# ambicuity/Distributed-LLM-Training-and-Inference-System

Hardware: AMD Instinct MI355X
Metric: tokens/sec (node) GPT-7B train (higher is better)
Workload: dtype bf16; 1 GPU; model=gpt-7b, global_batch=16, seq_len=2048, parallelism=dp1, micro_batch=16, grad_accum=1, activation_checkpoint=none, layout=planner

## Files before the change

### llmctl/config/knobs.py

```python

from __future__ import annotations

import contextlib
import dataclasses
import os
from dataclasses import dataclass, fields
from typing import Any, Dict, Iterator, Optional

ENV = "LLMCTL_KNOBS"


@dataclass(frozen=True)
class PerfKnobs:
    gemm64: bool = True
    gemm64_config: int = 304
    fwd64: str = "auto"
    dgrad64: str = "fused"
    wgrad_kernel: bool = True
    swiglu_bwd: str = "side"
    dgrad_transpose: bool = True
    wt_side_stream: bool = True
    fused_fwd: bool = False
    rope_inplace: bool = True
    fused_rope_attn: bool = True
    moe_pad: bool = True
    overlap_optimizer: bool = False
    gemm_tuning: bool = True
    fa_split: int = -1
    fa_prio: int = 1
    fa_nw: int = 4
    dkv: int = 2
    dkv_nwg: int = 0
    async_tp: bool = True
    async_tp_save_full: bool = False
    cp_zigzag: bool = True
    decode_fused: bool = True
    decode_splits: int = 0
    decode_v3: int = 1
    skinny_gemm: str = "auto"
    prefill_swiglu: bool = True
    prefill_fa: bool = True
    prefill_norm_fold: bool = True
    mixed_steps: bool = True
    custom_ar: bool = True
    tp_graphs: bool = True
    async_decode: bool = True
    tp_fused_decode: bool = True

    def as_dict(self) -> Dict[str, Any]:
        return dataclasses.asdict(self)


NATIVE = ("fa_split", "fa_prio", "fa_nw", "dkv", "dkv_nwg", "decode_splits", "decode_v3")
_FIELDS = {f.name: f for f in fields(PerfKnobs)}


def _coerce(name: str, value: Any) -> Any:
    if name not in _FIELDS:
        raise KeyError(f"unknown performance knob {name!r} (known: {', '.join(sorted(_FIELDS))})")
    typ = _FIELDS[name].type
    if typ in ("bool", bool):
        if isinstance(value, str):
            v = value.strip().lower()
            if v not in ("1", "0", "true", "false", "on", "off", "yes", "no"):
                raise ValueError(f"knob {name}: expected a boolean, got {value!r}")
            return v in ("1", "true", "on", "yes")
        return bool(value)
    if typ in ("int", int):
        return int(value)
    return str(value)


def parse_env(spec: Optional[str]) -> Dict[str, Any]:
    out: Dict[str, Any] = {}
    for part in (spec or "").split(","):
        part = part.strip()
        if not part:
            continue
        if "=" not in part:
            raise ValueError(f"{ENV}: expected name=value, got {part!r}")
        k, v = part.split("=", 1)
        out[k.strip()] = _coerce(k.strip(), v.strip())
    return out


_RETIRED_ENV = ("LLMCTL_SIDE_DGRAD", "LLMCTL_DECODE_ATTN_QKV", "LLMCTL_GEMM64_CONFIG", "LLMCTL_SKINNY")
_warned: set = set()


def _warn_retired_env() -> None:
    import warnings

    names = [f"LLMCTL_{n.upper()}" for n in _FIELDS] + list(_RETIRED_ENV)
    for n in names:
        if n in os.environ and n not in _warned:
            _warned.add(n)
            warnings.warn(f"{n} is no longer read (performance switches are knobs now): set "
                          f"{ENV}=\"{n[7:].lower()}=<value>\" or the [perf] config table instead", stacklevel=3)


def resolve(overrides: Optional[Dict[str, Any]] = None, env: bool = True) -> PerfKnobs:
    _warn_retired_env()
    kw = {k: _coerce(k, v) for k, v in (overrides or {}).items()}
    if env:
        kw.update(parse_env(os.environ.get(ENV)))
    return PerfKnobs(**kw)
# ... 57 lines not shown
```

### llmctl/ops/csrc/attn_common.h

```cpp
#pragma once
#include "common.h"

namespace llmctl {
namespace attn {

using bf16x8_t = __attribute__((ext_vector_type(8))) __bf16;
using s4_t = __attribute__((ext_vector_type(4))) short;
using s8_t = __attribute__((ext_vector_type(8))) short;
using f32x16 = __attribute__((ext_vector_type(16))) float;
using lds_s4 = __attribute__((address_space(3))) s4_t;

__device__ __forceinline__ f32x16 mfma32(bf16x8_t a, bf16x8_t b, f32x16 c) {
  return __builtin_amdgcn_mfma_f32_32x32x16_bf16(a, b, c, 0, 0, 0);
}

__device__ __forceinline__ float fast_exp2(float x) { return __builtin_amdgcn_exp2f(x); }

__device__ __forceinline__ float xor32_max(float x) {
  const auto r = __builtin_amdgcn_permlane32_swap(__float_as_uint(x), __float_as_uint(x), false, false);
  return fmaxf(__uint_as_float(r[0]), __uint_as_float(r[1]));
}
__device__ __forceinline__ float xor32_add(float x) {
  const auto r = __builtin_amdgcn_permlane32_swap(__float_as_uint(x), __float_as_uint(x), false, false);
  return __uint_as_float(r[0]) + __uint_as_float(r[1]);
// ... 26 lines not shown
}

template <int HD>
__device__ __forceinline__ bf16x8_t tr_frag(const unsigned char* base, int row0, int col0, int lane) {
  const int h = lane >> 5;
  const int i16 = lane & 15;
  const int q = i16 >> 2, p = i16 & 3;
  const int col = col0 + 16 * ((lane >> 4) & 1) + 4 * p;
  const int chunk = col >> 3;
  const int sub = (col & 7) * 2;
  const int r1 = row0 + 4 * h + q;
  const int r2 = r1 + 8;
  s4_t lo = __builtin_amdgcn_ds_read_tr16_b64_v4i16((lds_s4*)(base + tr_off<HD>(r1, chunk) + sub));
  s4_t hi = __builtin_amdgcn_ds_read_tr16_b64_v4i16((lds_s4*)(base + tr_off<HD>(r2, chunk) + sub));
  s8_t v = {lo[0], lo[1], lo[2], lo[3], hi[0], hi[1], hi[2], hi[3]};
  return __builtin_bit_cast(bf16x8_t, v);
}

template <int HD>
__device__ __forceinline__ void tr_frag_offs(int col0, int lane, int& lo, int& hi) {
  const int h = lane >> 5;
  const int i16 = lane & 15;
  const int q = i16 >> 2, p = i16 & 3;
  const int col = col0 + 16 * ((lane >> 4) & 1) + 4 * p;
  const int chunk = col >> 3;
  const int sub = (col & 7) * 2;
  lo = tr_off<HD>(4 * h + q, chunk) + sub;
  hi = tr_off<HD>(8 + 4 * h + q, chunk) + sub;
}
template <int HD>
__device__ __forceinline__ bf16x8_t tr_frag_at(const unsigned char* base, int row0, int lo, int hi) {
  s4_t a = __builtin_amdgcn_ds_read_tr16_b64_v4i16((lds_s4*)(base + row0 * (HD * 2) + lo));
  s4_t b = __builtin_amdgcn_ds_read_tr16_b64_v4i16((lds_s4*)(base + row0 * (HD * 2) + hi));
  s8_t v = {a[0], a[1], a[2], a[3], b[0], b[1], b[2], b[3]};
  return __builtin_bit_cast(bf16x8_t, v);
}

template <int HD>
__device__ __forceinline__ bf16x8_t tr_frag_nat(const unsigned char* base, int row0, int col0, int lane) {
  const int h = lane >> 5;
  const int i16 = lane & 15;
  const int q = i16 >> 2, p = i16 & 3;
  const int col = col0 + 16 * ((lane >> 4) & 1) + 4 * p;
  const int chunk = col >> 3;
  const int sub = (col & 7) * 2;
  const int r1 = row0 + 8 * h + q;
  const int r2 = r1 + 4;
  s4_t lo = __builtin_amdgcn_ds_read_tr16_b64_v4i16((lds_s4*)(base + tr_off<HD>(r1, chunk) + sub));
  s4_t hi = __builtin_amdgcn_ds_read_tr16_b64_v4i16((lds_s4*)(base + tr_off<HD>(r2, chunk) + sub));
  s8_t v = {lo[0], lo[1], lo[2], lo[3], hi[0], hi[1], hi[2], hi[3]};
  return __builtin_bit_cast(bf16x8_t, v);
}

__device__ __forceinline__ bf16x8_t to_bf16x8(const float* x) {
  bf16x8_t v;
#pragma unroll
  for (int j = 0; j < 8; ++j) v[j] = (__bf16)x[j];
  return v;
}

__device__ __forceinline__ uint4 gload16(const unsigned short* p) { return *reinterpret_cast<const uint4*>(p); }

__device__ __forceinline__ void dma16(const void* g, unsigned lds_byte) {
  asm volatile("s_mov_b32 m0, %1\n\ts_nop 0\n\tglobal_load_lds_dwordx4 %0, off" ::"v"(g), "s"(lds_byte) : "memory");
}
__device__ __forceinline__ void dma4(const void* g, unsigned lds_byte) {
  asm volatile("s_mov_b32 m0, %1\n\ts_nop 0\n\tglobal_load_lds_dword %0, off" ::"v"(g), "s"(lds_byte) : "memory");
}
template <int N>
__device__ __forceinline__ void vm_wait() {
  static_assert(N >= 0 && N <= 15, "vmcnt immediate");
  if constexpr (N == 0) asm volatile("s_waitcnt vmcnt(0)" ::: "memory");
  else if constexpr (N == 5) asm volatile("s_waitcnt vmcnt(5)" ::: "memory");
  else if constexpr (N == 9) asm volatile("s_waitcnt vmcnt(9)" ::: "memory");
  else static_assert(N == 0 || N == 5 || N == 9, "add the immediate");
}
using i32x4_t = __attribute__((ext_vector_type(4))) int;
__device__ __forceinline__ i32x4_t buf_rsrc(const void* base, unsigned num_records) {
  const unsigned long a = (unsigned long)base;
  i32x4_t r;
  r[0] = __builtin_amdgcn_readfirstlane((int)(a & 0xffffffffu));
  r[1] = __builtin_amdgcn_readfirstlane((int)((a >> 32) & 0xffff));
  r[2] = __builtin_amdgcn_readfirstlane((int)num_records);
  r[3] = 0x00020000;
  return r;
}
__device__ __forceinline__ void buf_dma16(i32x4_t rsrc, unsigned voff, unsigned lds_byte) {
  asm volatile("s_mov_b32 m0, %2\n\ts_nop 0\n\tbuffer_load_dwordx4 %0, %1, 0 offen lds" ::"v"(voff), "s"(rsrc),
               "s"(lds_byte)
               : "memory");
}
__device__ __forceinline__ void buf_dma4(i32x4_t rsrc, unsigned voff, unsigned lds_byte) {
  asm volatile("s_mov_b32 m0, %2\n\ts_nop 0\n\tbuffer_load_dword %0, %1, 0 offen lds" ::"v"(voff), "s"(rsrc),
               "s"(lds_byte)
               : "memory");
}
template <int N>
__device__ __forceinline__ void vm_wait_n() {
  static_assert(N >= 0 && N <= 63, "vmcnt immediate");
  asm volatile("s_waitcnt vmcnt(%0)" ::"i"(N) : "memory");
}

__device__ __forceinline__ unsigned lds_addr(const void* p) {
  return __builtin_amdgcn_readfirstlane(
      (unsigned)(uintptr_t)(const __attribute__((address_space(3))) unsigned char*)p);
}
// ... 4 lines not shown
```

### llmctl/ops/csrc/flash_attn_bwd.hip

```cpp
#include <cstdlib>
#include <map>
#include <mutex>

#include "attn_common.h"

namespace llmctl {
using namespace attn;
namespace {

constexpr float LOG2E = 1.4426950408889634f;
constexpr int KV_KB = 128;
constexpr int KV_QT = 64;
#ifndef LLMCTL_DKV_NBUF
#define LLMCTL_DKV_NBUF 2
#endif
constexpr int KV_NBUF = LLMCTL_DKV_NBUF;
static_assert(KV_NBUF >= 2 && KV_NBUF <= 4, "dK/dV ring depth 2-4");
constexpr int DQ_QB = 128;
constexpr int DQ_KB = 64;

struct BwdArgs {
  const unsigned short *q, *k, *v, *dout;
  const float* lse;
  const float* delta;
// ... 951 lines not shown
        w[0] = (unsigned)f2bf(x[0] * mul) | ((unsigned)f2bf(x[1] * mul) << 16);
        w[1] = (unsigned)f2bf(x[2] * mul) | ((unsigned)f2bf(x[3] * mul) << 16);
        asm volatile("global_store_dwordx2 %0, %1, off" ::"v"(p), "v"(w) : "memory");
      };
#pragma unroll
      for (int d = 0; d < NDB / 2; ++d) {
        const f32x16 x1 = acc_copy(dk[d]), x2 = acc_copy(dk[d + NDB / 2]);
        acc_zero(dk[d]);
        acc_zero(dk[d + NDB / 2]);
#pragma unroll
        for (int g = 0; g < 4; ++g) {
          const int col = d * 32 + 8 * g + 4 * hh;
          float lo[4], hi[4];
#pragma unroll
          for (int j = 0; j < 4; ++j) {
            const float c1 = rope ? cs[d][g][j] : 1.f, s1 = rope ? sn[d][g][j] : 0.f;
            lo[j] = x1[4 * g + j] * c1 + x2[4 * g + j] * s1;
            hi[j] = x2[4 * g + j] * c1 - x1[4 * g + j] * s1;
          }
          st8(dkp + col, lo, a.scale);
          st8(dkp + col + HD / 2, hi, a.scale);
        }
      }
#pragma unroll
      for (int d = 0; d < NDB; ++d) {
        const f32x16 x = acc_copy(dv[d]);
        acc_zero(dv[d]);
#pragma unroll
        for (int g = 0; g < 4; ++g) {
          float y[4];
#pragma unroll
          for (int j = 0; j < 4; ++j) y[j] = x[4 * g + j];
          st8(dvp + d * 32 + 8 * g + 4 * hh, y, 1.f);
        }
      }
      load_kv(pend0 >= 0 ? pend0 : cur);
      asm volatile("s_waitcnt vmcnt(0)"
                   : "+a"(kf[0]), "+a"(kf[1]), "+a"(kf[2]), "+a"(kf[3]), "+a"(kf[4]), "+a"(kf[5]), "+a"(kf[6]),
                     "+a"(kf[7]), "+a"(vf[0]), "+a"(vf[1]), "+a"(vf[2]), "+a"(vf[3]), "+a"(vf[4]), "+a"(vf[5]),
                     "+a"(vf[6]), "+a"(vf[7])
                   :
                   : "memory");
    }
    stamp(2);
    ++n_done;
    if (pend0 < 0) break;
    cur = pend0;
    pend0 = pend1;
    pend1 = -1;
    --npend;
  }
}

template <int HD, bool CAUSAL, bool DOC>
__global__ __launch_bounds__(256, 2) void fa_bwd_dq_kernel(BwdArgs a) {
  constexpr int NKS = HD / 16;
  constexpr int NDB = HD / 32;
  constexpr int ROWB = HD * 2;
  constexpr int TILE = DQ_KB * ROWB;
  constexpr int PPW = TILE / 1024 / 4;
  constexpr int SLOT = 2 * TILE;
  __shared__ __attribute__((aligned(1024))) unsigned char smem[2 * SLOT];

  const int tid = threadIdx.x;
  const int lane = tid & 63;
  const int wave = __builtin_amdgcn_readfirstlane(tid >> 6);
  const int r = lane & 31, hh = lane >> 5;
  const int nqb = (a.S + DQ_QB - 1) / DQ_QB;
  const int BH = a.B * a.Hq;
  int bh, qi;
  if (BH % 8) {
    bh = blockIdx.x % BH;
    qi = blockIdx.x / BH;
  } else {
    const int x = blockIdx.x & 7, j = blockIdx.x >> 3;
    bh = x * (BH >> 3) + j / nqb;
    qi = j % nqb;
  }
  const int qblk = nqb - 1 - qi;
  const int b = bh / a.Hq, hq = bh % a.Hq;
  const int hk = hq / (a.Hq / a.Hkv);
  const int q_row0 = qblk * DQ_QB + wave * 32;
  const int my_q = q_row0 + r;
  const int qc = min(my_q, a.S - 1);

  const unsigned short* Kp = a.k + b * a.k_sb + hk * a.k_sh;
  const unsigned short* Vp = a.v + b * a.v_sb + hk * a.v_sh;

#pragma unroll
  for (int i = 0; i < 2 * SLOT / 4096; ++i)
    *reinterpret_cast<uint4*>(smem + i * 4096 + tid * 16) = make_uint4(0, 0, 0, 0);

  bf16x8_t qf[NKS], df[NKS];
  {
    const unsigned short* Qp = a.q + b * a.q_sb + hq * a.q_sh + (long)qc * a.q_ss + 8 * hh;
    const unsigned short* Dp = a.dout + b * a.do_sb + hq * a.do_sh + (long)qc * a.do_ss + 8 * hh;
#pragma unroll
    for (int ks = 0; ks < NKS; ++ks) {
      qf[ks] = __builtin_bit_cast(bf16x8_t, gload16(Qp + 16 * ks));
      df[ks] = __builtin_bit_cast(bf16x8_t, gload16(Dp + 16 * ks));
    }
  }
  const long rc = ((long)b * a.Hq + hq) * a.S + qc;
  const float nlse2 = -a.lse[rc] * LOG2E;
  float dlt;
  if (a.o != nullptr) {
    const unsigned short* Op = a.o + b * a.o_sb + hq * a.o_sh + (long)qc * a.o_ss + 8 * hh;
// ... 24 lines not shown
    for (int i = 0; i < 16; ++i) dq[d][i] = 0.f;

  const int kv_end = CAUSAL ? min(a.S, qblk * DQ_QB + DQ_QB) : a.S;
  const int ntiles = (kv_end + DQ_KB - 1) / DQ_KB;
  int my_start = 0, w_min = 0, w_max = 0, t0 = 0;
  if constexpr (DOC) {
    const int* ds = a.doc + (long)b * a.S;
    my_start = ds[qc];
    w_min = __builtin_amdgcn_readfirstlane(ds[min(q_row0, a.S - 1)]);
    w_max = __builtin_amdgcn_readfirstlane(ds[min(q_row0 + 31, a.S - 1)]);
    t0 = __builtin_amdgcn_readfirstlane(ds[min(qblk * DQ_QB, a.S - 1)]) / DQ_KB;
  }
  const int key_hi = CAUSAL ? qc : a.S - 1;
  int klo[NDB], khi[NDB];
#pragma unroll
  for (int d = 0; d < NDB; ++d) tr_frag_offs<HD>(d * 32, lane, klo[d], khi[d]);
  int kro[NKS], vro[NKS];
#pragma unroll
  for (int ks = 0; ks < NKS; ++ks) {
    kro[ks] = tr_off<HD>(r, 2 * ks + hh);
    vro[ks] = row_off<HD>(r, 2 * ks + hh);
  }

  unsigned vk[PPW], vv[PPW];
#pragma unroll
  for (int i = 0; i < PPW; ++i) {
    const int byte = (i * 4 + wave) * 1024 + lane * 16;
    const int row = byte / ROWB, pch = (byte % ROWB) >> 4;
    vk[i] = (unsigned)((row * a.k_ss + ((pch ^ swz_tr<HD>(row)) << 3)) * 2);
    vv[i] = (unsigned)((row * a.v_ss + ((pch ^ swz_row<HD>(row)) << 3)) * 2);
  }
  const unsigned lds0 = lds_addr(smem);
  int ik0 = t0 * DQ_KB;
  const unsigned short* kc = Kp + (long)ik0 * a.k_ss;
  const unsigned short* vc = Vp + (long)ik0 * a.v_ss;
  const long k_step = (long)DQ_KB * a.k_ss, v_step = (long)DQ_KB * a.v_ss;
  auto issue = [&](auto slot_c) __attribute__((always_inline)) {
    constexpr int SLC = decltype(slot_c)::value;
    const int nk = min(DQ_KB, a.S - ik0);
    i32x4_t rk = buf_rsrc(kc, (unsigned)(((nk - 1) * a.k_ss + HD) * 2));
    i32x4_t rv = buf_rsrc(vc, (unsigned)(((nk - 1) * a.v_ss + HD) * 2));
    asm volatile("s_nop 4" : "+s"(rk), "+s"(rv));
    const unsigned slot = lds0 + (unsigned)(SLC * SLOT) + wave * 1024;
#pragma unroll
    for (int i = 0; i < PPW; ++i) {
      buf_dma16(rk, vk[i], slot + i * 4096);
      buf_dma16(rv, vv[i], slot + TILE + i * 4096);
    }
    ik0 += DQ_KB;
    kc += k_step;
    vc += v_step;
  };

  auto tile = [&](bool need_mask, const unsigned char* Ks, const unsigned char* Vs, int kv0)
                  __attribute__((always_inline)) {
#pragma unroll
    for (int kb = 0; kb < 2; ++kb) {
      f32x16 s, dp;
#pragma unroll
      for (int i = 0; i < 16; ++i) s[i] = dp[i] = 0.f;
#pragma unroll
      for (int ks = 0; ks < NKS; ++ks) {
        s = mfma32(lds_read_b128(Ks, kb * 32 * (HD * 2) + kro[ks]), qf[ks], s);
        dp = mfma32(lds_read_b128(Vs, kb * 32 * (HD * 2) + vro[ks]), df[ks], dp);
      }
      if (need_mask) {
#pragma unroll
        for (int i = 0; i < 16; ++i) {
          const int key = kv0 + kb * 32 + acc_row(i, hh);
          bool ok = key <= key_hi;
          if constexpr (DOC) ok = ok && key >= my_start;
          s[i] = ok ? s[i] : -INFINITY;
        }
      }
      float dsv[16];
#pragma unroll
      for (int i = 0; i < 16; ++i) dsv[i] = fast_exp2(__builtin_fmaf(s[i], a.scale_log2, nlse2)) * (dp[i] - dlt);
#pragma unroll
      for (int st = 0; st < 2; ++st) {
        const bf16x8_t sbf = to_bf16x8(dsv + 8 * st);
#pragma unroll
        for (int d = 0; d < NDB; ++d) dq[d] = mfma32(tr_frag_at<HD>(Ks, kb * 32 + 16 * st, klo[d], khi[d]), sbf, dq[d]);
      }
    }
  };

  __syncthreads();
  auto step = [&](auto slot_c, int t) __attribute__((always_inline)) {
    constexpr int SL = decltype(slot_c)::value;
    vm_wait_n<0>();
    __builtin_amdgcn_s_barrier();
    if (t + 1 < ntiles) issue(std::integral_constant<int, 1 - SL>{});
    const int kv0 = t * DQ_KB;
    bool live = true;
    if constexpr (CAUSAL) live = kv0 <= q_row0 + 31;
    if constexpr (DOC) live = live && kv0 + DQ_KB > w_min;
    if (live) {
      const bool need_mask =
          (CAUSAL && kv0 + DQ_KB - 1 > q_row0) || (kv0 + DQ_KB > a.S) || (DOC && kv0 < w_max);
      tile(need_mask, smem + SL * SLOT, smem + SL * SLOT + TILE, kv0);
    }
  };
  if (t0 < ntiles) issue(std::integral_constant<int, 0>{});
  for (int t = t0; t < ntiles; t += 2) {
    step(std::integral_constant<int, 0>{}, t);
    if (t + 1 < ntiles) step(std::integral_constant<int, 1>{}, t + 1);
  }
  if (my_q < a.S) {
    const long tok = (long)b * a.S + my_q;
    const float *cr = nullptr, *sr = nullptr;
    if (a.cos_t != nullptr) {
      const long p = a.rope_pos ? (long)a.rope_pos[tok] : tok % a.rope_S;
      cr = a.cos_t + p * (HD / 2);
      sr = a.sin_t + p * (HD / 2);
    }
    store_row<HD>(a.dq + tok * a.dq_st + (long)hq * HD, dq, a.scale, hh, cr, sr);
  }
}

int dkv_mode() {
  const int64_t m = knob("dkv", 2);
  return (m >= 0 && m <= 2) ? (int)m : 2;
}

int* dkv_queue(hipStream_t s) {
  static std::mutex mu;
  static std::map<std::pair<int, hipStream_t>, int*> bufs;
  int dev = 0;
  LLMCTL_HIP_CHECK(hipGetDevice(&dev));
  std::lock_guard<std::mutex> lk(mu);
  int*& q = bufs[{dev, s}];
  if (q == nullptr) LLMCTL_HIP_CHECK(hipMalloc(&q, 64 * sizeof(int)));
  return q;
}

template <int HD, bool CAUSAL, bool DOC>
void launch_bwd(const BwdArgs& a, hipStream_t s, bool do_dq, bool do_dkv, int dkv_impl) {
  if (do_dq) {
    const int nqb = (a.S + DQ_QB - 1) / DQ_QB;
    hipLaunchKernelGGL((fa_bwd_dq_kernel<HD, CAUSAL, DOC>), dim3((unsigned)(a.B * a.Hq * nqb)), dim3(256), 0, s, a);
  }
  if (do_dkv) {
    const int nkb = (a.S + KV_KB - 1) / KV_KB;
    const dim3 grid((unsigned)(a.B * a.Hkv * nkb));
    if constexpr (HD == 128 && CAUSAL) {
      if (dkv_impl == 2 && a.stamps != nullptr) {
        hipLaunchKernelGGL((fa_bwd_dkv_pipe_kernel<HD, CAUSAL, DOC, true>), grid, dim3(256), 0, s, a);
        return;
      }
      if constexpr (!DOC) {
        if (a.S % KV_KB == 0 && (dkv_impl == 3 || dkv_impl == 4 || (dkv_impl < 0 && dkv_mode() == 2))) {
          int* wq = dkv_queue(s);
          LLMCTL_HIP_CHECK(hipMemsetAsync(wq, 0, 8 * sizeof(int), s));
          int nwg = std::min<long>((long)num_cus(), (long)a.B * a.Hkv * nkb);
          const int min_wg = ((long)a.B * a.Hkv) % 8 == 0 ? 8 : 1;
          if (const int64_t e = knob("dkv_nwg", 0); e > 0) nwg = std::max<int>(min_wg, std::min<int>(nwg, (int)e));
          nwg = std::max(nwg, min_wg);
          if (a.stamps != nullptr)
            hipLaunchKernelGGL(fa_bwd_dkv_persist_kernel<true>, dim3((unsigned)nwg), dim3(256), 0, s, a, wq);
          else
            hipLaunchKernelGGL(fa_bwd_dkv_persist_kernel<false>, dim3((unsigned)nwg), dim3(256), 0, s, a, wq);
          return;
        }
      }
      if (dkv_impl == 1 || dkv_impl == 3 || (dkv_impl < 0 && dkv_mode() >= 1)) {
        hipLaunchKernelGGL((fa_bwd_dkv_pipe_kernel<HD, CAUSAL, DOC>), grid, dim3(256), 0, s, a);
        return;
      }
    }
    hipLaunchKernelGGL((fa_bwd_dkv_kernel<HD, CAUSAL, DOC>), grid, dim3(256), 0, s, a);
  }
}

void dispatch_bwd(const BwdArgs& a, int D, bool causal, bool doc, hipStream_t s, bool do_dq = true,
                  bool do_dkv = true, int dkv_impl = -1) {
  if (doc) {
    if (D == 128) launch_bwd<128, true, true>(a, s, do_dq, do_dkv, dkv_impl);
    else launch_bwd<64, true, true>(a, s, do_dq, do_dkv, dkv_impl);
  } else if (D == 128) {
    if (causal) launch_bwd<128, true, false>(a, s, do_dq, do_dkv, dkv_impl);
    else launch_bwd<128, false, false>(a, s, do_dq, do_dkv, dkv_impl);
  } else {
    if (causal) launch_bwd<64, true, false>(a, s, do_dq, do_dkv, dkv_impl);
    else launch_bwd<64, false, false>(a, s, do_dq, do_dkv, dkv_impl);
  }
}

BwdArgs make_args(const at::Tensor& dout, const at::Tensor& q, const at::Tensor& k, const at::Tensor& v,
                  const at::Tensor& lse, const at::Tensor& delta, at::Tensor& dq, at::Tensor& dk, at::Tensor& dv,
                  double scale) {
  return BwdArgs{bf_ptr(q), bf_ptr(k), bf_ptr(v), bf_ptr(dout), lse.data_ptr<float>(), delta.data_ptr<float>(),
                 bf_mut(dq), bf_mut(dk), bf_mut(dv), (int)q.size(0), (int)q.size(1), (int)q.size(2),
                 (int)k.size(2), q.stride(0), q.stride(1), q.stride(2), k.stride(0), k.stride(1), k.stride(2),
// ... 156 lines not shown
```

### llmctl/ops/csrc/flash_attn_fwd.hip

```cpp
#include <cstdlib>

#include "attn_common.h"

namespace llmctl {
using namespace attn;
namespace {

constexpr int KB = 64;
constexpr float kRescaleTh = 8.f;

struct FwdArgs {
  const unsigned short* q;
  const unsigned short* k;
  const unsigned short* v;
  unsigned short* o;
  float* lse;
  int B, S, Hq, Hkv;
  long q_sb, q_ss, q_sh;
  long k_sb, k_ss, k_sh;
  long v_sb, v_ss, v_sh;
  long o_sb, o_ss, o_sh;
  float scale_log2;
  const int* doc;
  unsigned short* o_part;
  float* lse_part;
  int prio;
};

template <int HD, bool CAUSAL, bool DOC = false, bool SPLIT = false, int NW = 4, int NBUF = 2>
__global__ __launch_bounds__(NW * 64, 2) void fa_fwd_kernel(FwdArgs a) {
  constexpr int QB = NW * 32;
  constexpr int NTHR = NW * 64;
  constexpr int NKS = HD / 16;
  constexpr int NDB = HD / 32;
  constexpr int ROWB = HD * 2;
  constexpr int TILE = KB * ROWB;
  constexpr int PPW = TILE / 1024 / NW;
  constexpr int SLOT = 2 * TILE;
  static_assert(PPW * NW * 1024 == TILE, "pieces must split evenly over the waves");
  __shared__ __attribute__((aligned(1024))) unsigned char smem[NBUF * SLOT];

  const int tid = threadIdx.x;
  const int lane = tid & 63;
  const int wave = __builtin_amdgcn_readfirstlane(tid >> 6);
  const int r = lane & 31, hh = lane >> 5;
  const int nqb = (a.S + QB - 1) / QB;
  const int BH = a.B * a.Hq;
  int bh, rest;
  if (SPLIT || BH % 8) {
    bh = blockIdx.x % BH;
    rest = blockIdx.x / BH;
  } else {
    const int x = blockIdx.x & 7, j = blockIdx.x >> 3;
    bh = x * (BH >> 3) + j / nqb;
    rest = j % nqb;
  }
  const int part = SPLIT ? rest & 1 : 0;
  const int qblk = nqb - 1 - (SPLIT ? rest >> 1 : rest);
  const int b = bh / a.Hq, hq = bh % a.Hq;
  const int hk = hq / (a.Hq / a.Hkv);
  const int q_row0 = qblk * QB + wave * 32;
  const int my_q = q_row0 + r;

  const unsigned short* Qp = a.q + b * a.q_sb + hq * a.q_sh;
  const unsigned short* Kp = a.k + b * a.k_sb + hk * a.k_sh;
  const unsigned short* Vp = a.v + b * a.v_sb + hk * a.v_sh;

#pragma unroll
  for (int i = 0; i < NBUF * SLOT / (NTHR * 16); ++i)
    *reinterpret_cast<uint4*>(smem + i * NTHR * 16 + tid * 16) = make_uint4(0, 0, 0, 0);

  bf16x8_t qf[NKS];
#pragma unroll
  for (int ks = 0; ks < NKS; ++ks) {
    uint4 u = make_uint4(0, 0, 0, 0);
    if (my_q < a.S) u = gload16(Qp + (long)my_q * a.q_ss + ks * 16 + 8 * hh);
    qf[ks] = __builtin_bit_cast(bf16x8_t, u);
  }

  f32x16 o[NDB];
#pragma unroll
  for (int d = 0; d < NDB; ++d)
// ... 7 lines not shown
  if constexpr (DOC) {
    const int* ds = a.doc + (long)b * a.S;
    my_start = ds[min(my_q, a.S - 1)];
    w_min = __builtin_amdgcn_readfirstlane(ds[min(q_row0, a.S - 1)]);
    w_max = __builtin_amdgcn_readfirstlane(ds[min(q_row0 + 31, a.S - 1)]);
    t0 = __builtin_amdgcn_readfirstlane(ds[min(qblk * QB, a.S - 1)]) / KB;
  }
  if constexpr (SPLIT) {
    const int mid = (t0 + ntiles) / 2;
    if (part == 0) ntiles = mid;
    else t0 = mid;
  }

  unsigned vk[PPW], vv[PPW];
#pragma unroll
  for (int i = 0; i < PPW; ++i) {
    const int byte = (i * NW + wave) * 1024 + lane * 16;
    const int row = byte / ROWB, pch = (byte % ROWB) >> 4;
    vk[i] = (unsigned)((row * a.k_ss + ((pch ^ swz_row<HD>(row)) << 3)) * 2);
    vv[i] = (unsigned)((row * a.v_ss + ((pch ^ swz_tr<HD>(row)) << 3)) * 2);
  }
  const unsigned lds0 = lds_addr(smem);
  int ik0 = t0 * KB;
  const unsigned short* kc = Kp + (long)ik0 * a.k_ss;
  const unsigned short* vc = Vp + (long)ik0 * a.v_ss;
  const long k_step = (long)KB * a.k_ss, v_step = (long)KB * a.v_ss;
  auto issue = [&](auto slot_c) __attribute__((always_inline)) {
    constexpr int SLC = decltype(slot_c)::value;
    const int nk = min(KB, a.S - ik0);
    i32x4_t rk = buf_rsrc(kc, (unsigned)(((nk - 1) * a.k_ss + HD) * 2));
    i32x4_t rv = buf_rsrc(vc, (unsigned)(((nk - 1) * a.v_ss + HD) * 2));
    asm volatile("s_nop 4" : "+s"(rk), "+s"(rv));
    const unsigned slot = lds0 + (unsigned)(SLC * SLOT) + wave * 1024;
#pragma unroll
    for (int i = 0; i < PPW; ++i) {
      buf_dma16(rk, vk[i], slot + i * NW * 1024);
      buf_dma16(rv, vv[i], slot + TILE + i * NW * 1024);
    }
    ik0 += KB;
    kc += k_step;
    vc += v_step;
  };

  const float c = a.scale_log2;
  const int key_hi = CAUSAL ? min(my_q, a.S - 1) : a.S - 1;
  int vlo[NDB], vhi[NDB];
#pragma unroll
  for (int d = 0; d < NDB; ++d) tr_frag_offs<HD>(d * 32, lane, vlo[d], vhi[d]);
  int kofs[NKS];
#pragma unroll
  for (int ks = 0; ks < NKS; ++ks) kofs[ks] = row_off<HD>(r, 2 * ks + hh);
#pragma unroll
  for (int ks = 0; ks < NKS; ++ks) asm volatile("" ::"v"(qf[ks]));
  auto tile = [&](bool need_mask, const unsigned char* Ks, const unsigned char* Vs, int kv0) __attribute__((always_inline)) {
    if (a.prio) __builtin_amdgcn_s_setprio(1);
    f32x16 s[2];
#pragma unroll
    for (int kb = 0; kb < 2; ++kb) {
#pragma unroll
      for (int i = 0; i < 16; ++i) s[kb][i] = 0.f;
#pragma unroll
      for (int ks = 0; ks < NKS; ++ks) s[kb] = mfma32(lds_read_b128(Ks, kb * 32 * (HD * 2) + kofs[ks]), qf[ks], s[kb]);
    }
    if (need_mask) {
#pragma unroll
      for (int kb = 0; kb < 2; ++kb)
#pragma unroll
        for (int i = 0; i < 16; ++i) {
          const int key = kv0 + kb * 32 + acc_row(i, hh);
          bool ok = key <= key_hi;
          if constexpr (DOC) ok = ok && key >= my_start;
          s[kb][i] = ok ? s[kb][i] : -INFINITY;
        }
    }
    if (a.prio) __builtin_amdgcn_s_setprio(0);
    float mx = s[0][0];
#pragma unroll
    for (int kb = 0; kb < 2; ++kb)
#pragma unroll
      for (int i = (kb == 0 ? 1 : 0); i < 16; ++i) mx = fmaxf(mx, s[kb][i]);
    mx = xor32_max(mx) * c;
    const bool grow = __builtin_amdgcn_ballot_w64(mx > m_i + kRescaleTh) != 0;
    const float m_new = grow ? fmaxf(m_i, mx) : m_i;
    const float nm = (m_new == -INFINITY) ? 0.f : -m_new;
    float rs = 0.f;
    bf16x8_t pb[2][2];
#pragma unroll
    for (int kb = 0; kb < 2; ++kb) {
      float p[16];
#pragma unroll
      for (int i = 0; i < 16; ++i) {
        p[i] = fast_exp2(__builtin_fmaf(s[kb][i], c, nm));
        rs += p[i];
      }
      pb[kb][0] = to_bf16x8(p);
      pb[kb][1] = to_bf16x8(p + 8);
    }
    rs = xor32_add(rs);
    if (grow) {
      const float alpha = fast_exp2(m_i + nm);
      l_i *= alpha;
#pragma unroll
      for (int d = 0; d < NDB; ++d)
#pragma unroll
        for (int i = 0; i < 16; ++i) o[d][i] *= alpha;
    }
    l_i += rs;
    m_i = m_new;
    if (a.prio) __builtin_amdgcn_s_setprio(1);
#pragma unroll
    for (int kb = 0; kb < 2; ++kb)
#pragma unroll
      for (int st = 0; st < 2; ++st)
#pragma unroll
        for (int d = 0; d < NDB; ++d) o[d] = mfma32(tr_frag_at<HD>(Vs, kb * 32 + 16 * st, vlo[d], vhi[d]), pb[kb][st], o[d]);
    if (a.prio) __builtin_amdgcn_s_setprio(0);
  };

  __syncthreads();
  auto step = [&](auto slot_c, int t) __attribute__((always_inline)) {
    constexpr int SL = decltype(slot_c)::value;
    if constexpr (NBUF == 3) {
      if (t + 1 < ntiles) vm_wait_n<2 * PPW>();
      else vm_wait_n<0>();
    } else {
      vm_wait_n<0>();
    }
    __builtin_amdgcn_s_barrier();
    if (t + NBUF - 1 < ntiles) issue(std::integral_constant<int, (SL + NBUF - 1) % NBUF>{});
    const int kv0 = t * KB;
    bool live = true;
    if constexpr (CAUSAL) live = kv0 <= q_row0 + 31;
    if constexpr (DOC) live = live && kv0 + KB > w_min;
    if (live) {
      const bool need_mask = (CAUSAL && kv0 + KB - 1 > q_row0) || (kv0 + KB > a.S) || (DOC && kv0 < w_max);
      tile(need_mask, smem + SL * SLOT, smem + SL * SLOT + TILE, kv0);
    }
  };
  if (t0 < ntiles) issue(std::integral_constant<int, 0>{});
  if constexpr (NBUF == 3)
    if (t0 + 1 < ntiles) issue(std::integral_constant<int, 1>{});
  for (int t = t0; t < ntiles; t += NBUF) {
    step(std::integral_constant<int, 0>{}, t);
    if (t + 1 < ntiles) step(std::integral_constant<int, 1>{}, t + 1);
    if constexpr (NBUF == 3)
      if (t + 2 < ntiles) step(std::integral_constant<int, 2>{}, t + 2);
  }

  if constexpr (SPLIT) {
    if (my_q < a.S) {
      const float inv = l_i > 0.f ? 1.f / l_i : 0.f;
      unsigned short* Op = a.o_part + ((((long)part * a.B + b) * a.S + my_q) * a.Hq + hq) * HD;
#pragma unroll
      for (int d = 0; d < NDB; ++d)
#pragma unroll
        for (int g = 0; g < 4; ++g) {
          const int col = d * 32 + 8 * g + 4 * hh;
          unsigned short w4[4];
#pragma unroll
          for (int j = 0; j < 4; ++j) w4[j] = f2bf(o[d][4 * g + j] * inv);
          *reinterpret_cast<uint2*>(Op + col) =
              make_uint2((unsigned)w4[0] | ((unsigned)w4[1] << 16), (unsigned)w4[2] | ((unsigned)w4[3] << 16));
        }
      if (hh == 0)
        a.lse_part[(((long)part * a.B + b) * a.Hq + hq) * a.S + my_q] =
            (l_i > 0.f) ? (m_i + __log2f(l_i)) * 0.69314718055994531f : -INFINITY;
    }
    return;
  }
  if (my_q < a.S) {
    const float inv = l_i > 0.f ? 1.f / l_i : 0.f;
    unsigned short* Op = a.o + b * a.o_sb + (long)my_q * a.o_ss + hq * a.o_sh;
#pragma unroll
    for (int d = 0; d < NDB; ++d)
#pragma unroll
      for (int g = 0; g < 4; ++g) {
        const int col = d * 32 + 8 * g + 4 * hh;
        unsigned short w4[4];
#pragma unroll
        for (int j = 0; j < 4; ++j) w4[j] = f2bf(o[d][4 * g + j] * inv);
        *reinterpret_cast<uint2*>(Op + col) =
            make_uint2((unsigned)w4[0] | ((unsigned)w4[1] << 16), (unsigned)w4[2] | ((unsigned)w4[3] << 16));
      }
    if (hh == 0) {
      const float lse = (l_i > 0.f) ? (m_i + __log2f(l_i)) * 0.69314718055994531f : -INFINITY;
      a.lse[((long)b * a.Hq + hq) * a.S + my_q] = lse;
    }
  }
}

template <int HD>
__global__ __launch_bounds__(256) void fa_combine_kernel(const unsigned short* __restrict__ o_part,
                                                         const float* __restrict__ lse_part,
                                                         unsigned short* __restrict__ o, float* __restrict__ lse,
                                                         int B, int S, int Hq, long o_sb, long o_ss, long o_sh) {
  constexpr int LPR = HD / 8;
  const long gid = (long)blockIdx.x * 256 + threadIdx.x;
  const long row = gid / LPR;
  const int sub = gid % LPR;
  if (row >= (long)B * S * Hq) return;
  const int hq = row % Hq;
  const long bs = row / Hq;
  const int sq = bs % S;
  const int b = bs / S;
  const long li = ((long)b * Hq + hq) * S + sq;
  const long plane = (long)B * Hq * S;
  const float l0 = lse_part[li], l1 = lse_part[plane + li];
  const float m = fmaxf(l0, l1);
  float w0 = 0.f, w1 = 0.f, l = -INFINITY;
  if (m != -INFINITY) {
    const float e0 = __expf(l0 - m), e1 = __expf(l1 - m);
    l = m + __logf(e0 + e1);
    w0 = e0 / (e0 + e1);
    w1 = e1 / (e0 + e1);
  }
  const long ob = row * HD + sub * 8;
  const long osz = (long)B * S * Hq * HD;
  float out[8], x0[8], x1[8];
  load8(o_part + ob, x0);
  load8(o_part + osz + ob, x1);
#pragma unroll
  for (int j = 0; j < 8; ++j) out[j] = w0 * x0[j] + w1 * x1[j];
  store8(o + b * o_sb + (long)sq * o_ss + (long)hq * o_sh + sub * 8, out);
  if (sub == 0) lse[li] = l;
}

template <int NW, int NBUF>
std::tuple<at::Tensor, at::Tensor> fwd_launch(const at::Tensor& q, at::Tensor& o, at::Tensor& lse, FwdArgs& a, int B,
                                              int S, int Hq, int D, bool causal,
                                              const c10::optional<at::Tensor>& doc_start) {
  constexpr int QB = NW * 32, WG_PER_CU = NW == 4 ? 2 : 1;
  const int nqb = (S + QB - 1) / QB;
  dim3 grid((unsigned)(B * Hq * nqb)), block(NW * 64);
  auto s = stream();
  bool split = causal && !(doc_start.has_value() && doc_start->defined()) && nqb >= 4 &&
               (long)B * Hq * nqb <= (long)WG_PER_CU * num_cus();
  if (const int64_t e = knob("fa_split", -1); e == 0) split = false;
  else if (e == 1) split = causal && !(doc_start.has_value() && doc_start->defined()) && nqb >= 2;
  if (split) {
    auto o_part = at::empty({2, B, S, Hq, D}, q.options());
    auto lse_part = at::empty({2, B, Hq, S}, q.options().dtype(at::kFloat));
    a.o_part = bf_mut(o_part);
    a.lse_part = lse_part.data_ptr<float>();
    dim3 g2((unsigned)(2 * B * Hq * nqb));
    const long threads = (long)B * S * Hq * (D / 8);
    if (D == 128) {
      hipLaunchKernelGGL((fa_fwd_kernel<128, true, false, true, NW, NBUF>), g2, block, 0, s, a);
      hipLaunchKernelGGL(fa_combine_kernel<128>, dim3((threads + 255) / 256), dim3(256), 0, s, a.o_part, a.lse_part,
                         bf_mut(o), lse.data_ptr<float>(), B, S, Hq, o.stride(0), o.stride(1), o.stride(2));
    } else {
      hipLaunchKernelGGL((fa_fwd_kernel<64, true, false, true, NW, NBUF>), g2, block, 0, s, a);
      hipLaunchKernelGGL(fa_combine_kernel<64>, dim3((threads + 255) / 256), dim3(256), 0, s, a.o_part, a.lse_part,
                         bf_mut(o), lse.data_ptr<float>(), B, S, Hq, o.stride(0), o.stride(1), o.stride(2));
    }
    return {o, lse};
  }
  if (doc_start.has_value() && doc_start->defined()) {
    const at::Tensor& ds = *doc_start;
    LLMCTL_CHECK(causal, "flash_attn_fwd: doc_start (packed sequences) needs causal attention");
    LLMCTL_CHECK(ds.is_cuda() && ds.scalar_type() == at::kInt && ds.is_contiguous() && ds.dim() == 2 &&
                     ds.size(0) == B && ds.size(1) == S,
                 "flash_attn_fwd: doc_start must be contiguous int32 [B,S]");
    a.doc = ds.data_ptr<int>();
    if (D == 128) hipLaunchKernelGGL((fa_fwd_kernel<128, true, true, false, NW, NBUF>), grid, block, 0, s, a);
    else hipLaunchKernelGGL((fa_fwd_kernel<64, true, true, false, NW, NBUF>), grid, block, 0, s, a);
    return {o, lse};
  }
  if (D == 128) {
    if (causal) hipLaunchKernelGGL((fa_fwd_kernel<128, true, false, false, NW, NBUF>), grid, block, 0, s, a);
    else hipLaunchKernelGGL((fa_fwd_kernel<128, false, false, false, NW, NBUF>), grid, block, 0, s, a);
  } else {
    if (causal) hipLaunchKernelGGL((fa_fwd_kernel<64, true, false, false, NW, NBUF>), grid, block, 0, s, a);
    else hipLaunchKernelGGL((fa_fwd_kernel<64, false, false, false, NW, NBUF>), grid, block, 0, s, a);
  }
  return {o, lse};
}

}

std::tuple<at::Tensor, at::Tensor> flash_attn_fwd(const at::Tensor& q, const at::Tensor& k, const at::Tensor& v,
                                                  double scale, bool causal,
                                                  const c10::optional<at::Tensor>& doc_start) {
  LLMCTL_CHECK(q.is_cuda() && k.is_cuda() && v.is_cuda(), "flash_attn_fwd: GPU tensors");
  LLMCTL_CHECK(q.scalar_type() == at::kBFloat16 && k.scalar_type() == at::kBFloat16 &&
                   v.scalar_type() == at::kBFloat16,
               "flash_attn_fwd: bf16");
  LLMCTL_CHECK(q.dim() == 4 && k.dim() == 4 && v.dim() == 4, "q/k/v must be [B,S,H,D]");
  const int B = q.size(0), S = q.size(1), Hq = q.size(2), D = q.size(3);
  const int Hkv = k.size(2);
  LLMCTL_CHECK(k.size(0) == B && k.size(1) == S && v.sizes() == k.sizes() && k.size(3) == D,
               "k/v shape must be [B,S,Hkv,D] matching q");
  LLMCTL_CHECK(Hq % Hkv == 0, "Hq must be a multiple of Hkv");
  LLMCTL_CHECK(D == 64 || D == 128, "head_dim must be 64 or 128, got ", D);
  LLMCTL_CHECK(q.stride(3) == 1 && k.stride(3) == 1 && v.stride(3) == 1, "head_dim must be contiguous");
  for (const at::Tensor* t : {&q, &k, &v})
    LLMCTL_CHECK(t->stride(0) % 8 == 0 && t->stride(1) % 8 == 0 && t->stride(2) % 8 == 0 &&
                     (reinterpret_cast<uintptr_t>(t->data_ptr()) & 15) == 0,
                 "q/k/v strides must be multiples of 8 elements and 16-B aligned");
  const c10::DeviceGuard g(q.device());
  auto o = at::empty({B, S, Hq, D}, q.options());
  auto lse = at::empty({B, Hq, S}, q.options().dtype(at::kFloat));
  if (B * S * Hq == 0) return {o, lse};
  FwdArgs a{bf_ptr(q), bf_ptr(k), bf_ptr(v), bf_mut(o), lse.data_ptr<float>(), B, S, Hq, Hkv,
            q.stride(0), q.stride(1), q.stride(2), k.stride(0), k.stride(1), k.stride(2),
            v.stride(0), v.stride(1), v.stride(2), o.stride(0), o.stride(1), o.stride(2),
            (float)(scale * 1.4426950408889634), nullptr, nullptr, nullptr, 0};
  a.prio = knob("fa_prio", 1) != 0 ? 1 : 0;
  if (knob("fa_nw", 4) == 8) return fwd_launch<8, 3>(q, o, lse, a, B, S, Hq, D, causal, doc_start);
  return fwd_launch<4, 2>(q, o, lse, a, B, S, Hq, D, causal, doc_start);
}

TORCH_LIBRARY_IMPL(llmctl, CUDA, m) { m.impl("flash_attn_fwd", &flash_attn_fwd); }

}
```

Baseline: 30920 tokens/s.

## Software-pipeline LDS fragment reads against MFMAs in flash-attention forward and dQ kernels

Adds a register ring that prefetches K and V LDS fragments one step ahead of the MFMA that consumes them in the flash-attention forward kernel, with sched_group_barrier hints to interleave the reads with MFMAs. The first K fragments of a tile are loaded before the next tile's global prefetch is issued. An equivalent pipelining is added to the backward dQ kernel behind a knob bit that is off by default. The aim is to hide LDS read latency behind matrix math, at the cost of extra VGPR pressure under launch_bounds(…,2).

```diff
diff --git a/llmctl/config/knobs.py b/llmctl/config/knobs.py
--- a/llmctl/config/knobs.py
+++ b/llmctl/config/knobs.py
@@ -29,6 +29,7 @@
     fa_split: int = -1
     fa_prio: int = 1
     fa_nw: int = 4
+    fa_frag_prefetch: int = 1
     dkv: int = 2
     dkv_nwg: int = 0
     async_tp: bool = True
@@ -51,7 +52,7 @@
         return dataclasses.asdict(self)
 
 
-NATIVE = ("fa_split", "fa_prio", "fa_nw", "dkv", "dkv_nwg", "decode_splits", "decode_v3")
+NATIVE = ("fa_split", "fa_prio", "fa_nw", "fa_frag_prefetch", "dkv", "dkv_nwg", "decode_splits", "decode_v3")
 _FIELDS = {f.name: f for f in fields(PerfKnobs)}
 
 
diff --git a/llmctl/ops/csrc/attn_common.h b/llmctl/ops/csrc/attn_common.h
--- a/llmctl/ops/csrc/attn_common.h
+++ b/llmctl/ops/csrc/attn_common.h
@@ -102,6 +102,12 @@
   return __builtin_bit_cast(bf16x8_t, v);
 }
 
+template <int NMFMA, int NREAD>
+__device__ __forceinline__ void sched_mfma_reads() {
+  __builtin_amdgcn_sched_group_barrier(0x008, NMFMA, 0);
+  __builtin_amdgcn_sched_group_barrier(0x100, NREAD, 0);
+}
+
 __device__ __forceinline__ bf16x8_t to_bf16x8(const float* x) {
   bf16x8_t v;
 #pragma unroll
diff --git a/llmctl/ops/csrc/flash_attn_bwd.hip b/llmctl/ops/csrc/flash_attn_bwd.hip
--- a/llmctl/ops/csrc/flash_attn_bwd.hip
+++ b/llmctl/ops/csrc/flash_attn_bwd.hip
@@ -1027,7 +1027,7 @@
   }
 }
 
-template <int HD, bool CAUSAL, bool DOC>
+template <int HD, bool CAUSAL, bool DOC, bool PF>
 __global__ __launch_bounds__(256, 2) void fa_bwd_dq_kernel(BwdArgs a) {
   constexpr int NKS = HD / 16;
   constexpr int NDB = HD / 32;
@@ -1158,6 +1158,17 @@
     vc += v_step;
   };
 
+  constexpr int PD = 2;
+  constexpr int HR = 2 * PD / NDB;
+  static_assert(NKS >= PD + 2 && NDB % 2 == 0 && HR * NDB == 2 * PD, "ring shape");
+  bf16x8_t kq[PD], vq[PD], tq[NDB];
+  auto sd_head = [&](const unsigned char* Ks, const unsigned char* Vs) __attribute__((always_inline)) {
+#pragma unroll
+    for (int p = 0; p < PD; ++p) {
+      kq[p] = lds_read_b128(Ks, kro[p]);
+      vq[p] = lds_read_b128(Vs, vro[p]);
+    }
+  };
   auto tile = [&](bool need_mask, const unsigned char* Ks, const unsigned char* Vs, int kv0)
                   __attribute__((always_inline)) {
 #pragma unroll
@@ -1165,10 +1176,31 @@
       f32x16 s, dp;
 #pragma unroll
       for (int i = 0; i < 16; ++i) s[i] = dp[i] = 0.f;
-#pragma unroll
-      for (int ks = 0; ks < NKS; ++ks) {
-        s = mfma32(lds_read_b128(Ks, kb * 32 * (HD * 2) + kro[ks]), qf[ks], s);
-        dp = mfma32(lds_read_b128(Vs, kb * 32 * (HD * 2) + vro[ks]), df[ks], dp);
+      if constexpr (PF) {
+#pragma unroll
+        for (int ks = 0; ks < NKS; ++ks) {
+          s = mfma32(kq[ks % PD], qf[ks], s);
+          dp = mfma32(vq[ks % PD], df[ks], dp);
+          if (ks + PD < NKS) {
+            kq[ks % PD] = lds_read_b128(Ks, kb * 32 * (HD * 2) + kro[ks + PD]);
+            vq[ks % PD] = lds_read_b128(Vs, kb * 32 * (HD * 2) + vro[ks + PD]);
+            sched_mfma_reads<2, 2>();
+          }
+          if (ks + 2 >= NKS) {
+#pragma unroll
+            for (int i = 0; i < NDB / 2; ++i) {
+              const int d = (ks + 2 - NKS) * (NDB / 2) + i;
+              tq[d] = tr_frag_at<HD>(Ks, kb * 32, klo[d], khi[d]);
+            }
+            sched_mfma_reads<2, NDB>();
+          }
+        }
+      } else {
+#pragma unroll
+        for (int ks = 0; ks < NKS; ++ks) {
+          s = mfma32(lds_read_b128(Ks, kb * 32 * (HD * 2) + kro[ks]), qf[ks], s);
+          dp = mfma32(lds_read_b128(Vs, kb * 32 * (HD * 2) + vro[ks]), df[ks], dp);
+        }
       }
       if (need_mask) {
 #pragma unroll
@@ -1185,8 +1217,26 @@
 #pragma unroll
       for (int st = 0; st < 2; ++st) {
         const bf16x8_t sbf = to_bf16x8(dsv + 8 * st);
-#pragma unroll
-        for (int d = 0; d < NDB; ++d) dq[d] = mfma32(tr_frag_at<HD>(Ks, kb * 32 + 16 * st, klo[d], khi[d]), sbf, dq[d]);
+        if constexpr (PF) {
+#pragma unroll
+          for (int d = 0; d < NDB; ++d) {
+            dq[d] = mfma32(tq[d], sbf, dq[d]);
+            if (st == 0) {
+              tq[d] = tr_frag_at<HD>(Ks, kb * 32 + 16, klo[d], khi[d]);
+              sched_mfma_reads<1, 2>();
+            } else if (kb == 0) {
+#pragma unroll
+              for (int i = d * HR; i < (d + 1) * HR; ++i) {
+                if (i % 2 == 0) kq[i / 2] = lds_read_b128(Ks, 32 * (HD * 2) + kro[i / 2]);
+                else vq[i / 2] = lds_read_b128(Vs, 32 * (HD * 2) + vro[i / 2]);
+              }
+              sched_mfma_reads<1, HR>();
+            }
+          }
+        } else {
+#pragma unroll
+          for (int d = 0; d < NDB; ++d) dq[d] = mfma32(tr_frag_at<HD>(Ks, kb * 32 + 16 * st, klo[d], khi[d]), sbf, dq[d]);
+        }
       }
     }
   };
@@ -1196,11 +1246,16 @@
     constexpr int SL = decltype(slot_c)::value;
     vm_wait_n<0>();
     __builtin_amdgcn_s_barrier();
-    if (t + 1 < ntiles) issue(std::integral_constant<int, 1 - SL>{});
+    if constexpr (!PF)
+      if (t + 1 < ntiles) issue(std::integral_constant<int, 1 - SL>{});
     const int kv0 = t * DQ_KB;
     bool live = true;
     if constexpr (CAUSAL) live = kv0 <= q_row0 + 31;
     if constexpr (DOC) live = live && kv0 + DQ_KB > w_min;
+    if constexpr (PF) {
+      if (live) sd_head(smem + SL * SLOT, smem + SL * SLOT + TILE);
+      if (t + 1 < ntiles) issue(std::integral_constant<int, 1 - SL>{});
+    }
     if (live) {
       const bool need_mask =
           (CAUSAL && kv0 + DQ_KB - 1 > q_row0) || (kv0 + DQ_KB > a.S) || (DOC && kv0 < w_max);
@@ -1244,7 +1299,11 @@
 void launch_bwd(const BwdArgs& a, hipStream_t s, bool do_dq, bool do_dkv, int dkv_impl) {
   if (do_dq) {
     const int nqb = (a.S + DQ_QB - 1) / DQ_QB;
-    hipLaunchKernelGGL((fa_bwd_dq_kernel<HD, CAUSAL, DOC>), dim3((unsigned)(a.B * a.Hq * nqb)), dim3(256), 0, s, a);
+    const dim3 grid((unsigned)(a.B * a.Hq * nqb));
+    if ((knob("fa_frag_prefetch", 1) & 2) != 0)
+      hipLaunchKernelGGL((fa_bwd_dq_kernel<HD, CAUSAL, DOC, true>), grid, dim3(256), 0, s, a);
+    else
+      hipLaunchKernelGGL((fa_bwd_dq_kernel<HD, CAUSAL, DOC, false>), grid, dim3(256), 0, s, a);
   }
   if (do_dkv) {
     const int nkb = (a.S + KV_KB - 1) / KV_KB;
diff --git a/llmctl/ops/csrc/flash_attn_fwd.hip b/llmctl/ops/csrc/flash_attn_fwd.hip
--- a/llmctl/ops/csrc/flash_attn_fwd.hip
+++ b/llmctl/ops/csrc/flash_attn_fwd.hip
@@ -27,7 +27,7 @@
   int prio;
 };
 
-template <int HD, bool CAUSAL, bool DOC = false, bool SPLIT = false, int NW = 4, int NBUF = 2>
+template <int HD, bool CAUSAL, bool DOC = false, bool SPLIT = false, int NW = 4, int NBUF = 2, bool PF = true>
 __global__ __launch_bounds__(NW * 64, 2) void fa_fwd_kernel(FwdArgs a) {
   constexpr int QB = NW * 32;
   constexpr int NTHR = NW * 64;
@@ -141,15 +141,40 @@
   for (int ks = 0; ks < NKS; ++ks) kofs[ks] = row_off<HD>(r, 2 * ks + hh);
 #pragma unroll
   for (int ks = 0; ks < NKS; ++ks) asm volatile("" ::"v"(qf[ks]));
+  bf16x8_t fr[NKS];
+  static_assert(2 * NDB == NKS, "one 32-key half of V has as many fragments as K has k-steps");
+  auto k_head = [&](const unsigned char* Ks) __attribute__((always_inline)) {
+#pragma unroll
+    for (int ks = 0; ks < NKS; ++ks) fr[ks] = lds_read_b128(Ks, kofs[ks]);
+  };
   auto tile = [&](bool need_mask, const unsigned char* Ks, const unsigned char* Vs, int kv0) __attribute__((always_inline)) {
     if (a.prio) __builtin_amdgcn_s_setprio(1);
     f32x16 s[2];
-#pragma unroll
-    for (int kb = 0; kb < 2; ++kb) {
-#pragma unroll
-      for (int i = 0; i < 16; ++i) s[kb][i] = 0.f;
-#pragma unroll
-      for (int ks = 0; ks < NKS; ++ks) s[kb] = mfma32(lds_read_b128(Ks, kb * 32 * (HD * 2) + kofs[ks]), qf[ks], s[kb]);
+    if constexpr (PF) {
+#pragma unroll
+      for (int kb = 0; kb < 2; ++kb)
+#pragma unroll
+        for (int i = 0; i < 16; ++i) s[kb][i] = 0.f;
+#pragma unroll
+      for (int ks = 0; ks < NKS; ++ks) {
+        s[0] = mfma32(fr[ks], qf[ks], s[0]);
+        fr[ks] = lds_read_b128(Ks, 32 * (HD * 2) + kofs[ks]);
+        sched_mfma_reads<1, 1>();
+      }
+#pragma unroll
+      for (int ks = 0; ks < NKS; ++ks) {
+        s[1] = mfma32(fr[ks], qf[ks], s[1]);
+        fr[ks] = tr_frag_at<HD>(Vs, 16 * (ks / NDB), vlo[ks % NDB], vhi[ks % NDB]);
+        sched_mfma_reads<1, 2>();
+      }
+    } else {
+#pragma unroll
+      for (int kb = 0; kb < 2; ++kb) {
+#pragma unroll
+        for (int i = 0; i < 16; ++i) s[kb][i] = 0.f;
+#pragma unroll
+        for (int ks = 0; ks < NKS; ++ks) s[kb] = mfma32(lds_read_b128(Ks, kb * 32 * (HD * 2) + kofs[ks]), qf[ks], s[kb]);
+      }
     }
     if (need_mask) {
 #pragma unroll
@@ -197,12 +222,23 @@
     l_i += rs;
     m_i = m_new;
     if (a.prio) __builtin_amdgcn_s_setprio(1);
-#pragma unroll
-    for (int kb = 0; kb < 2; ++kb)
-#pragma unroll
-      for (int st = 0; st < 2; ++st)
-#pragma unroll
-        for (int d = 0; d < NDB; ++d) o[d] = mfma32(tr_frag_at<HD>(Vs, kb * 32 + 16 * st, vlo[d], vhi[d]), pb[kb][st], o[d]);
+    if constexpr (PF) {
+#pragma unroll
+      for (int j = 0; j < NKS; ++j) {
+        o[j % NDB] = mfma32(fr[j], pb[0][j / NDB], o[j % NDB]);
+        fr[j] = tr_frag_at<HD>(Vs, 32 + 16 * (j / NDB), vlo[j % NDB], vhi[j % NDB]);
+        sched_mfma_reads<1, 2>();
+      }
+#pragma unroll
+      for (int j = 0; j < NKS; ++j) o[j % NDB] = mfma32(fr[j], pb[1][j / NDB], o[j % NDB]);
+    } else {
+#pragma unroll
+      for (int kb = 0; kb < 2; ++kb)
+#pragma unroll
+        for (int st = 0; st < 2; ++st)
+#pragma unroll
+          for (int d = 0; d < NDB; ++d) o[d] = mfma32(tr_frag_at<HD>(Vs, kb * 32 + 16 * st, vlo[d], vhi[d]), pb[kb][st], o[d]);
+    }
     if (a.prio) __builtin_amdgcn_s_setprio(0);
   };
 
@@ -216,11 +252,16 @@
       vm_wait_n<0>();
     }
     __builtin_amdgcn_s_barrier();
-    if (t + NBUF - 1 < ntiles) issue(std::integral_constant<int, (SL + NBUF - 1) % NBUF>{});
+    if constexpr (!PF)
+      if (t + NBUF - 1 < ntiles) issue(std::integral_constant<int, (SL + NBUF - 1) % NBUF>{});
     const int kv0 = t * KB;
     bool live = true;
     if constexpr (CAUSAL) live = kv0 <= q_row0 + 31;
     if constexpr (DOC) live = live && kv0 + KB > w_min;
+    if constexpr (PF) {
+      if (live) k_head(smem + SL * SLOT);
+      if (t + NBUF - 1 < ntiles) issue(std::integral_constant<int, (SL + NBUF - 1) % NBUF>{});
+    }
     if (live) {
       const bool need_mask = (CAUSAL && kv0 + KB - 1 > q_row0) || (kv0 + KB > a.S) || (DOC && kv0 < w_max);
       tile(need_mask, smem + SL * SLOT, smem + SL * SLOT + TILE, kv0);
@@ -314,7 +355,7 @@
   if (sub == 0) lse[li] = l;
 }
 
-template <int NW, int NBUF>
+template <int NW, int NBUF, bool PF>
 std::tuple<at::Tensor, at::Tensor> fwd_launch(const at::Tensor& q, at::Tensor& o, at::Tensor& lse, FwdArgs& a, int B,
                                               int S, int Hq, int D, bool causal,
                                               const c10::optional<at::Tensor>& doc_start) {
@@ -334,11 +375,11 @@
     dim3 g2((unsigned)(2 * B * Hq * nqb));
     const long threads = (long)B * S * Hq * (D / 8);
     if (D == 128) {
-      hipLaunchKernelGGL((fa_fwd_kernel<128, true, false, true, NW, NBUF>), g2, block, 0, s, a);
+      hipLaunchKernelGGL((fa_fwd_kernel<128, true, false, true, NW, NBUF, PF>), g2, block, 0, s, a);
       hipLaunchKernelGGL(fa_combine_kernel<128>, dim3((threads + 255) / 256), dim3(256), 0, s, a.o_part, a.lse_part,
                          bf_mut(o), lse.data_ptr<float>(), B, S, Hq, o.stride(0), o.stride(1), o.stride(2));
     } else {
-      hipLaunchKernelGGL((fa_fwd_kernel<64, true, false, true, NW, NBUF>), g2, block, 0, s, a);
+      hipLaunchKernelGGL((fa_fwd_kernel<64, true, false, true, NW, NBUF, PF>), g2, block, 0, s, a);
       hipLaunchKernelGGL(fa_combine_kernel<64>, dim3((threads + 255) / 256), dim3(256), 0, s, a.o_part, a.lse_part,
                          bf_mut(o), lse.data_ptr<float>(), B, S, Hq, o.stride(0), o.stride(1), o.stride(2));
     }
@@ -351,16 +392,16 @@
                      ds.size(0) == B && ds.size(1) == S,
                  "flash_attn_fwd: doc_start must be contiguous int32 [B,S]");
     a.doc = ds.data_ptr<int>();
-    if (D == 128) hipLaunchKernelGGL((fa_fwd_kernel<128, true, true, false, NW, NBUF>), grid, block, 0, s, a);
-    else hipLaunchKernelGGL((fa_fwd_kernel<64, true, true, false, NW, NBUF>), grid, block, 0, s, a);
+    if (D == 128) hipLaunchKernelGGL((fa_fwd_kernel<128, true, true, false, NW, NBUF, PF>), grid, block, 0, s, a);
+    else hipLaunchKernelGGL((fa_fwd_kernel<64, true, true, false, NW, NBUF, PF>), grid, block, 0, s, a);
     return {o, lse};
   }
   if (D == 128) {
-    if (causal) hipLaunchKernelGGL((fa_fwd_kernel<128, true, false, false, NW, NBUF>), grid, block, 0, s, a);
-    else hipLaunchKernelGGL((fa_fwd_kernel<128, false, false, false, NW, NBUF>), grid, block, 0, s, a);
+    if (causal) hipLaunchKernelGGL((fa_fwd_kernel<128, true, false, false, NW, NBUF, PF>), grid, block, 0, s, a);
+    else hipLaunchKernelGGL((fa_fwd_kernel<128, false, false, false, NW, NBUF, PF>), grid, block, 0, s, a);
   } else {
-    if (causal) hipLaunchKernelGGL((fa_fwd_kernel<64, true, false, false, NW, NBUF>), grid, block, 0, s, a);
-    else hipLaunchKernelGGL((fa_fwd_kernel<64, false, false, false, NW, NBUF>), grid, block, 0, s, a);
+    if (causal) hipLaunchKernelGGL((fa_fwd_kernel<64, true, false, false, NW, NBUF, PF>), grid, block, 0, s, a);
+    else hipLaunchKernelGGL((fa_fwd_kernel<64, false, false, false, NW, NBUF, PF>), grid, block, 0, s, a);
   }
   return {o, lse};
 }
@@ -395,8 +436,12 @@
             v.stride(0), v.stride(1), v.stride(2), o.stride(0), o.stride(1), o.stride(2),
             (float)(scale * 1.4426950408889634), nullptr, nullptr, nullptr, 0};
   a.prio = knob("fa_prio", 1) != 0 ? 1 : 0;
-  if (knob("fa_nw", 4) == 8) return fwd_launch<8, 3>(q, o, lse, a, B, S, Hq, D, causal, doc_start);
-  return fwd_launch<4, 2>(q, o, lse, a, B, S, Hq, D, causal, doc_start);
+  const bool pf = (knob("fa_frag_prefetch", 1) & 1) != 0;
+  if (knob("fa_nw", 4) == 8)
+    return pf ? fwd_launch<8, 3, true>(q, o, lse, a, B, S, Hq, D, causal, doc_start)
+              : fwd_launch<8, 3, false>(q, o, lse, a, B, S, Hq, D, causal, doc_start);
+  return pf ? fwd_launch<4, 2, true>(q, o, lse, a, B, S, Hq, D, causal, doc_start)
+            : fwd_launch<4, 2, false>(q, o, lse, a, B, S, Hq, D, causal, doc_start);
 }
 
 TORCH_LIBRARY_IMPL(llmctl, CUDA, m) { m.impl("flash_attn_fwd", &flash_attn_fwd); }
```

New measurement: 30940 tokens/s (median of 4 runs). Within noise of the previous version (+0.1%).
